# bytedance/byteps

Measured on AMD Instinct MI355X. Metric: images/sec (whole node), higher is better.
Workload: dtype bf16; 1 GPU; model=resnet50, global_batch=64, seq_len=224, parallelism=dp1, graph=True, compression=none, cross_barrier=False

## Files before the change

byteps_amd/ops/csrc/bn.hip:

```cpp
#include <hip/hip_runtime.h>
#include <hip/hip_bf16.h>

#define BLOCK 256
#define MAX_GRID 2048

namespace {

using bf16 = __hip_bfloat16;
typedef short short8 __attribute__((ext_vector_type(8)));
typedef float float4v __attribute__((ext_vector_type(4)));

__device__ inline float bf2f(bf16 v) { return __bfloat162float(v); }
__device__ inline bf16 f2bf(float v) { return __float2bfloat16(v); }

struct F8 {
  float v[8];
  __device__ void zero() {
#pragma unroll
    for (int i = 0; i < 8; ++i) v[i] = 0.0f;
  }
};

__device__ inline void load8(const bf16* p, float* out) {
  short8 r = *reinterpret_cast<const short8*>(p);
  const bf16* e = reinterpret_cast<const bf16*>(&r);
#pragma unroll
  for (int i = 0; i < 8; ++i) out[i] = bf2f(e[i]);
}

__device__ inline void store8(bf16* p, const float* in) {
  short8 r;
  bf16* e = reinterpret_cast<bf16*>(&r);
#pragma unroll
  for (int i = 0; i < 8; ++i) e[i] = f2bf(in[i]);
  *reinterpret_cast<short8*>(p) = r;
}

#define RED_BLOCKS 1024


__global__ void bn_reduce_kernel(const bf16* __restrict__ x, long long M,
                                 int C, float* __restrict__ partial) {
  const int cpt = C >> 3;
  const int groups = max(1, BLOCK / cpt);
  const int t = threadIdx.x;
  const int g = t / cpt;
  const int c8 = t - g * cpt;
  __shared__ float lds[BLOCK * 8];

  F8 s, q;
  s.zero();
  q.zero();
  if (g < groups) {
    float vals[8];
    for (long long row = (long long)blockIdx.x * groups + g; row < M;
         row += (long long)gridDim.x * groups) {
      load8(x + row * C + (c8 << 3), vals);
#pragma unroll
      for (int i = 0; i < 8; ++i) {
        s.v[i] += vals[i];
        q.v[i] += vals[i] * vals[i];
      }
    }
  }
#pragma unroll
  for (int i = 0; i < 8; ++i) lds[t * 8 + i] = s.v[i];
  __syncthreads();
  if (g == 0 && c8 < cpt) {
    for (int gg = 1; gg < groups; ++gg)
#pragma unroll
      for (int i = 0; i < 8; ++i) s.v[i] += lds[(gg * cpt + c8) * 8 + i];
#pragma unroll
    for (int i = 0; i < 8; ++i)
      partial[(long long)((c8 << 3) + i) * RED_BLOCKS + blockIdx.x] = s.v[i];
  }
  __syncthreads();
#pragma unroll
  for (int i = 0; i < 8; ++i) lds[t * 8 + i] = q.v[i];
  __syncthreads();
  if (g == 0 && c8 < cpt) {
    for (int gg = 1; gg < groups; ++gg)
#pragma unroll
      for (int i = 0; i < 8; ++i) q.v[i] += lds[(gg * cpt + c8) * 8 + i];
#pragma unroll
    for (int i = 0; i < 8; ++i)
      partial[(long long)(C + (c8 << 3) + i) * RED_BLOCKS + blockIdx.x] =
          q.v[i];
  }
}

__device__ inline float wave_row_sum(const float* __restrict__ row,
                                     int nblocks) {
  const int lane = threadIdx.x & 63;
  float acc = 0.0f;
  for (int b = lane; b < nblocks; b += 64) acc += row[b];
#pragma unroll
  for (int off = 32; off > 0; off >>= 1) acc += __shfl_down(acc, off, 64);
  return acc;
}

inline int red_grid(long long M, int C) {
  int groups = BLOCK / (C >> 3);
  if (groups < 1) groups = 1;
  long long need = (M + groups - 1) / groups;
  long long work_cap = (M * (long long)C) / 49152;
  if (work_cap < 64) work_cap = 64;
  if (need > work_cap) need = work_cap;
  if (need < 1) need = 1;
  return (int)(need < RED_BLOCKS ? need : RED_BLOCKS);
}


__global__ void bn_finalize_kernel(const float* __restrict__ partial,
                                   long long M, int C, float eps,
                                   float momentum,
                                   float* __restrict__ mean_out,
                                   float* __restrict__ invstd_out,
                                   float* __restrict__ running_mean,
                                   float* __restrict__ running_var,
                                   int update_running, int nblocks) {
  int c = blockIdx.x;
  if (c >= C) return;
  float sum = wave_row_sum(partial + (long long)c * RED_BLOCKS, nblocks);
  float sumsq = wave_row_sum(partial + (long long)(C + c) * RED_BLOCKS,
                             nblocks);
  if (threadIdx.x != 0) return;
  float n = (float)M;
  float mean = sum / n;
  float var = sumsq / n - mean * mean;
  if (var < 0.0f) var = 0.0f;
  mean_out[c] = mean;
  invstd_out[c] = rsqrtf(var + eps);
  if (update_running) {
    float unbiased = (M > 1) ? var * n / (n - 1.0f) : var;
    running_mean[c] += momentum * (mean - running_mean[c]);
    running_var[c] += momentum * (unbiased - running_var[c]);
  }
}


template <bool RELU, bool RES>
__global__ void bn_fwd_apply_kernel(const bf16* __restrict__ x,
                                    const bf16* __restrict__ res,
                                    bf16* __restrict__ y, long long M, int C,
                                    const float* __restrict__ mean,
                                    const float* __restrict__ invstd,
                                    const float* __restrict__ gamma,
                                    const float* __restrict__ beta,
                                    unsigned char* __restrict__ mask) {
  const int cpt = C >> 3;
  const long long total = M * cpt;
  for (long long idx = (long long)blockIdx.x * BLOCK + threadIdx.x;
       idx < total; idx += (long long)gridDim.x * BLOCK) {
    const long long row = idx / cpt;
    const int c8 = (int)(idx - row * cpt);
    const int c0 = c8 << 3;
    const long long off = row * C + c0;
    float vals[8], rv[8];
    load8(x + off, vals);
    if (RES) load8(res + off, rv);
    unsigned char mbits = 0;
#pragma unroll
    for (int i = 0; i < 8; ++i) {
      float scale = gamma[c0 + i] * invstd[c0 + i];
      float v = (vals[i] - mean[c0 + i]) * scale + beta[c0 + i];
      if (RES) v += rv[i];
      if (RELU) {
        if (v > 0.0f) mbits |= (unsigned char)(1u << i);
        else v = 0.0f;
      }
      vals[i] = v;
    }
    store8(y + off, vals);
    if (RELU) mask[idx] = mbits;
  }
}


template <bool RELU>
__global__ void bn_bwd_reduce_kernel(const bf16* __restrict__ x,
                                     const bf16* __restrict__ dy,
                                     const unsigned char* __restrict__ mask,
                                     long long M,
                                     int C, const float* __restrict__ mean,
                                     const float* __restrict__ invstd,
                                     float* __restrict__ partial) {
  const int cpt = C >> 3;
  const int groups = max(1, BLOCK / cpt);
  const int t = threadIdx.x;
  const int g = t / cpt;
  const int c8 = t - g * cpt;
  __shared__ float lds[BLOCK * 8];

  F8 s1, s2;
  s1.zero();
  s2.zero();
  if (g < groups) {
    float xv[8], dv[8];
    for (long long row = (long long)blockIdx.x * groups + g; row < M;
         row += (long long)gridDim.x * groups) {
      const long long off = row * C + (c8 << 3);
      load8(x + off, xv);
      load8(dy + off, dv);
      const unsigned char mbits = RELU ? mask[row * cpt + c8] : 0;
#pragma unroll
      for (int i = 0; i < 8; ++i) {
        const int c = (c8 << 3) + i;
        float dz = RELU ? ((mbits >> i) & 1 ? dv[i] : 0.0f) : dv[i];
        float xhat = (xv[i] - mean[c]) * invstd[c];
        s1.v[i] += dz;
        s2.v[i] += dz * xhat;
      }
    }
  }
#pragma unroll
  for (int i = 0; i < 8; ++i) lds[t * 8 + i] = s1.v[i];
  __syncthreads();
  if (g == 0 && c8 < cpt) {
    for (int gg = 1; gg < groups; ++gg)
#pragma unroll
      for (int i = 0; i < 8; ++i) s1.v[i] += lds[(gg * cpt + c8) * 8 + i];
#pragma unroll
    for (int i = 0; i < 8; ++i)
      partial[(long long)((c8 << 3) + i) * RED_BLOCKS + blockIdx.x] =
          s1.v[i];
  }
  __syncthreads();
#pragma unroll
  for (int i = 0; i < 8; ++i) lds[t * 8 + i] = s2.v[i];
  __syncthreads();
  if (g == 0 && c8 < cpt) {
    for (int gg = 1; gg < groups; ++gg)
#pragma unroll
      for (int i = 0; i < 8; ++i) s2.v[i] += lds[(gg * cpt + c8) * 8 + i];
#pragma unroll
    for (int i = 0; i < 8; ++i)
      partial[(long long)(C + (c8 << 3) + i) * RED_BLOCKS + blockIdx.x] =
          s2.v[i];
  }
}

__global__ void bn_fold_kernel(const float* __restrict__ partial, int C,
                               float* __restrict__ sums2, int nblocks) {
  int row = blockIdx.x;
  if (row >= 2 * C) return;
  float acc = wave_row_sum(partial + (long long)row * RED_BLOCKS, nblocks);
  if (threadIdx.x == 0) sums2[row] = acc;
}


template <bool RELU, bool RES>
__global__ void bn_bwd_apply_kernel(const bf16* __restrict__ x,
                                    const bf16* __restrict__ dy,
                                    const unsigned char* __restrict__ mask,
                                    bf16* __restrict__ dx,
                                    bf16* __restrict__ dres, long long M,
                                    int C, const float* __restrict__ mean,
                                    const float* __restrict__ invstd,
                                    const float* __restrict__ gamma,
                                    const float* __restrict__ sums2) {
  const int cpt = C >> 3;
  const long long total = M * cpt;
  const float rn = 1.0f / (float)M;
  for (long long idx = (long long)blockIdx.x * BLOCK + threadIdx.x;
       idx < total; idx += (long long)gridDim.x * BLOCK) {
    const long long row = idx / cpt;
    const int c8 = (int)(idx - row * cpt);
    const int c0 = c8 << 3;
    const long long off = row * C + c0;
    float xv[8], dv[8], dzv[8];
    load8(x + off, xv);
    load8(dy + off, dv);
    const unsigned char mbits = RELU ? mask[idx] : 0;
#pragma unroll
    for (int i = 0; i < 8; ++i) {
      const int c = c0 + i;
      float dz = RELU ? ((mbits >> i) & 1 ? dv[i] : 0.0f) : dv[i];
      dzv[i] = dz;
      float xhat = (xv[i] - mean[c]) * invstd[c];
      dv[i] = gamma[c] * invstd[c] *
              (dz - sums2[c] * rn - xhat * sums2[C + c] * rn);
    }
    store8(dx + off, dv);
    if (RES) store8(dres + off, dzv);
  }
}

inline int grid_for_rows(long long M, int C) {
  int groups = max(1, BLOCK / (C >> 3));
  long long blocks = (M + groups - 1) / groups;
  return (int)(blocks < MAX_GRID ? (blocks > 0 ? blocks : 1) : MAX_GRID);
}

inline int grid_for_elems(long long elems) {
  long long blocks = (elems + BLOCK - 1) / BLOCK;
  return (int)(blocks < MAX_GRID ? (blocks > 0 ? blocks : 1) : MAX_GRID);
}

}

#define STREAM reinterpret_cast<hipStream_t>(stream)

extern "C" {

int bps_bn_red_blocks(void) { return RED_BLOCKS; }

int bps_bn_reduce(const void* x, long long M, int C, void* partial,
                  void* stream) {
  if ((C & 7) || C > 2048) return -1;
  hipLaunchKernelGGL(bn_reduce_kernel, dim3(red_grid(M, C)), dim3(BLOCK), 0,
                     STREAM, (const bf16*)x, M, C, (float*)partial);
  return (int)hipGetLastError();
}

int bps_bn_finalize(const void* sums, long long M, int C, float eps,
                    float momentum, void* mean_out, void* invstd_out,
                    void* running_mean, void* running_var, int update_running,
                    void* stream) {
  hipLaunchKernelGGL(bn_finalize_kernel, dim3(C), dim3(64), 0,
                     STREAM, (const float*)sums, M, C, eps, momentum,
                     (float*)mean_out, (float*)invstd_out,
                     (float*)running_mean, (float*)running_var,
                     update_running, red_grid(M, C));
  return (int)hipGetLastError();
}

int bps_bn_fwd_apply(const void* x, const void* res, void* y, long long M,
                     int C, const void* mean, const void* invstd,
                     const void* gamma, const void* beta, int relu,
                     void* mask, void* stream) {
  if ((C & 7) || C > 2048) return -1;
  if (relu && !mask) return -2;
  int g = grid_for_elems(M * (C >> 3));
#define LAUNCH_FWD(R, S)                                                    \
  hipLaunchKernelGGL((bn_fwd_apply_kernel<R, S>), dim3(g), dim3(BLOCK), 0,  \
                     STREAM, (const bf16*)x, (const bf16*)res, (bf16*)y, M, \
                     C, (const float*)mean, (const float*)invstd,           \
                     (const float*)gamma, (const float*)beta,               \
                     (unsigned char*)mask)
  if (relu && res) LAUNCH_FWD(true, true);
  else if (relu) LAUNCH_FWD(true, false);
  else if (res) LAUNCH_FWD(false, true);
  else LAUNCH_FWD(false, false);
#undef LAUNCH_FWD
  return (int)hipGetLastError();
}

int bps_bn_bwd_reduce(const void* x, const void* dy, const void* mask,
                      long long M, int C, const void* mean,
                      const void* invstd, void* partial, int relu,
                      void* stream) {
  if ((C & 7) || C > 2048) return -1;
  if (relu && !mask) return -2;
  int g = red_grid(M, C);
  if (relu)
    hipLaunchKernelGGL((bn_bwd_reduce_kernel<true>), dim3(g),
                       dim3(BLOCK), 0, STREAM, (const bf16*)x,
                       (const bf16*)dy, (const unsigned char*)mask, M, C,
                       (const float*)mean, (const float*)invstd,
                       (float*)partial);
  else
    hipLaunchKernelGGL((bn_bwd_reduce_kernel<false>), dim3(g),
                       dim3(BLOCK), 0, STREAM, (const bf16*)x,
                       (const bf16*)dy, (const unsigned char*)mask, M, C,
                       (const float*)mean, (const float*)invstd,
                       (float*)partial);
  return (int)hipGetLastError();
}

int bps_bn_fold(const void* partial, long long M, int C, void* sums2,
                void* stream) {
  hipLaunchKernelGGL(bn_fold_kernel, dim3(2 * C), dim3(64), 0, STREAM,
                     (const float*)partial, C, (float*)sums2,
                     red_grid(M, C));
  return (int)hipGetLastError();
}

int bps_bn_bwd_apply(const void* x, const void* dy, const void* mask,
                     void* dx,
                     void* dres, long long M, int C, const void* mean,
                     const void* invstd, const void* gamma, const void* sums2,
                     int relu, void* stream) {
  if ((C & 7) || C > 2048) return -1;
  if (relu && !mask) return -2;
  int g = grid_for_elems(M * (C >> 3));
#define LAUNCH_BWD(R, S)                                                     \
  hipLaunchKernelGGL((bn_bwd_apply_kernel<R, S>), dim3(g), dim3(BLOCK), 0,   \
                     STREAM, (const bf16*)x, (const bf16*)dy,                \
                     (const unsigned char*)mask, (bf16*)dx, (bf16*)dres,     \
                     M, C,                                                   \
                     (const float*)mean, (const float*)invstd,               \
                     (const float*)gamma, (const float*)sums2)
  if (relu && dres) LAUNCH_BWD(true, true);
  else if (relu) LAUNCH_BWD(true, false);
  else if (dres) LAUNCH_BWD(false, true);
  else LAUNCH_BWD(false, false);
#undef LAUNCH_BWD
  return (int)hipGetLastError();
}

}
```

byteps_amd/ops/csrc/core.cc:

```cpp

#include <pybind11/pybind11.h>
#include <pybind11/stl.h>

#include <cstdint>
#include <stdexcept>

namespace py = pybind11;

extern "C" {
int bps_scale(void* x, int64_t n, float alpha, int dtype, void* stream);
int bps_cast_scale_many(const void* desc_dev, int nseg, int64_t total_vec,
                        float alpha, int src_dtype, int dst_dtype,
                        void* stream);
int bps_cast_scale(void* dst, const void* src, int64_t n, float alpha,
                   int src_dtype, int dst_dtype, void* stream);
int bps_lt_gemm_bias(const void* X, const void* W, const void* bias,
                     void* Y, int64_t M, int64_t N, int64_t K,
                     void* stream);
int bps_lt_gemm_dgelu(const void* dY2, const void* W2, const void* aux,
                      void* dY1, int64_t M, int64_t H, int64_t I,
                      void* stream);
int bps_lt_gemm_wgrad(const void* dY, const void* X, void* dW, void* db,
                      int64_t M, int64_t N, int64_t K, void* stream);
int bps_lt_gemm_dgrad(const void* dY, const void* W, void* dX, int64_t M,
                      int64_t N, int64_t K, void* stream);
int bps_axpy(void* y, const void* x, int64_t n, float alpha, int dtype,
             void* stream);
int bps_nesterov(void* g, void* m, int64_t n, float mu, int dtype,
                 void* stream);
int bps_norm(const void* x, int64_t n, int mode, void* out, int dtype,
             void* stream);
int bps_onebit_compress(const void* x, int64_t n, void* bits, void* scale_sum,
                        void* stream);
int bps_onebit_decompress(const void* bits, const void* scale_sum, int64_t n,
                          void* out, void* stream);
int bps_onebit_error(const void* x, const void* bits, const void* scale_sum,
                     int64_t n, void* err, void* stream);
int bps_randomk_compress(const void* x, int64_t n, int64_t k, uint64_t seed,
                         void* idx, void* val, void* stream);
int bps_sparse_scatter(const void* idx, const void* val, int64_t k, void* out,
                       void* stream);
int bps_sparse_error_zero(const void* idx, int64_t k, void* err, void* stream);
int bps_sparse_gather(const void* x, const void* idx, int64_t k, void* val,
                      void* stream);
int bps_dithering_compress(const void* x, int64_t n, int s, uint64_t seed,
                           int natural, const void* norm, void* code,
                           void* stream);
int bps_dithering_decompress(const void* code, int64_t n, int s, int natural,
                             const void* norm, void* out, void* stream);
int bps_fp8_compress(const void* x, int64_t n, const void* amax, void* code,
                     void* stream);
int bps_fp8_decompress(const void* code, int64_t n, const void* amax,
                       void* out, void* stream);

int bps_bn_reduce(const void* x, long long M, int C, void* sums,
                  void* stream);
int bps_bn_finalize(const void* sums, long long M, int C, float eps,
                    float momentum, void* mean_out, void* invstd_out,
                    void* running_mean, void* running_var, int update_running,
                    void* stream);
int bps_bn_fwd_apply(const void* x, const void* res, void* y, long long M,
                     int C, const void* mean, const void* invstd,
                     const void* gamma, const void* beta, int relu,
                     void* mask, void* stream);
int bps_bn_bwd_reduce(const void* x, const void* dy, const void* mask,
                      long long M, int C, const void* mean,
                      const void* invstd, void* partial, int relu,
                      void* stream);
int bps_bn_fold(const void* partial, long long M, int C, void* sums2,
                void* stream);
int bps_bn_red_blocks(void);

int bps_ln_supported(int C);
int bps_ln_red_blocks(void);
int bps_ln_fwd(const void* x, const void* gamma, const void* beta, void* y,
               long long M, int C, float eps, void* mean, void* invstd,
               void* stream);
int bps_ln_bwd(const void* x, const void* dy, const void* gamma,
               const void* mean, const void* invstd, void* dx, long long M,
               int C, void* partial, void* stream);
int bps_ln_fold(const void* partial, long long M, int C, void* sums2,
                void* stream);
int bps_bn_bwd_apply(const void* x, const void* dy, const void* mask,
                     void* dx,
                     void* dres, long long M, int C, const void* mean,
                     const void* invstd, const void* gamma, const void* sums2,
                     int relu, void* stream);

int bps_cpu_sum(void* dst, const void* src, int64_t n, int dtype);
int bps_cpu_sum2(void* dst, const void* src1, const void* src2, int64_t n,
                 float alpha, int dtype);
int bps_cpu_copy(void* dst, const void* src, int64_t nbytes);
int bps_cpu_scale(void* x, int64_t n, float alpha, int dtype);
int bps_cpu_topk_select(const float* x, int64_t n, int64_t k, int32_t* idx,
                        float* val);
int bps_cpu_dither_encode(const int8_t* code, int64_t n, uint8_t* out,
                          int64_t out_cap, int64_t* out_len);
int bps_cpu_dither_decode(const uint8_t* in, int64_t in_len, int64_t n,
                          int8_t* code);
int bps_cpu_onebit_compress(const float* x, int64_t n, uint64_t* bits,
                            float* scale_sum);
int bps_cpu_onebit_decompress(const uint64_t* bits, float scale_sum, int64_t n,
                              float* out);
int bps_cpu_randomk_indices(int64_t n, int64_t k, uint64_t seed, int32_t* idx);
int bps_cpu_sparse_scatter(const int32_t* idx, const float* val, int64_t k,
                           float* out);
int bps_cpu_sparse_accumulate(const int32_t* idx, const float* val, int64_t k,
                              float* acc);
int bps_cpu_dithering_compress(const float* x, int64_t n, int s, uint64_t seed,
                               int natural, float norm, int8_t* code);
int bps_cpu_dithering_decompress(const int8_t* code, int64_t n, int s,
                                 int natural, float norm, float* out);
int bps_cpu_fp8_compress(const float* x, int64_t n, float amax,
                         uint8_t* code);
int bps_cpu_fp8_decompress(const uint8_t* code, int64_t n, float amax,
                           float* out);
float bps_cpu_norm(const float* x, int64_t n, int mode);
}

namespace {

inline void check(int rc, const char* what) {
  if (rc != 0)
    throw std::runtime_error(std::string(what) + " failed with code " +
                             std::to_string(rc));
}

#define P(x) reinterpret_cast<void*>(static_cast<uintptr_t>(x))
#define CP(x) reinterpret_cast<const void*>(static_cast<uintptr_t>(x))

}

void init_kv(py::module_& m);
void init_server(py::module_& m);

PYBIND11_MODULE(_core, m) {
  m.doc() = "byteps_amd native core: HIP gfx950 kernels, CPU reducer, KV";
  m.attr("HIP_KERNELS") = true;

  m.def("scale", [](uintptr_t x, int64_t n, float a, int dt, uintptr_t s) {
    check(bps_scale(P(x), n, a, dt, P(s)), "bps_scale");
  });
  m.def("axpy",
        [](uintptr_t y, uintptr_t x, int64_t n, float a, int dt, uintptr_t s) {
          check(bps_axpy(P(y), CP(x), n, a, dt, P(s)), "bps_axpy");
        });
  m.def("cast_scale_many",
        [](uintptr_t desc, int nseg, int64_t total_vec, float a, int sdt,
           int ddt, uintptr_t s) {
          check(bps_cast_scale_many(CP(desc), nseg, total_vec, a, sdt, ddt,
                                    P(s)), "bps_cast_scale_many");
        });
  m.def("cast_scale",
        [](uintptr_t dst, uintptr_t src, int64_t n, float a, int sdt,
// ... 36 lines not shown
        [](uintptr_t x, int64_t n, int mode, uintptr_t out, int dt,
           uintptr_t s) {
          check(bps_norm(CP(x), n, mode, P(out), dt, P(s)), "bps_norm");
        });
  m.def("onebit_compress",
        [](uintptr_t x, int64_t n, uintptr_t bits, uintptr_t sc, uintptr_t s) {
          check(bps_onebit_compress(CP(x), n, P(bits), P(sc), P(s)),
                "bps_onebit_compress");
        });
  m.def("onebit_decompress",
        [](uintptr_t bits, uintptr_t sc, int64_t n, uintptr_t out,
           uintptr_t s) {
          check(bps_onebit_decompress(CP(bits), CP(sc), n, P(out), P(s)),
                "bps_onebit_decompress");
        });
  m.def("onebit_error",
        [](uintptr_t x, uintptr_t bits, uintptr_t sc, int64_t n, uintptr_t err,
           uintptr_t s) {
          check(bps_onebit_error(CP(x), CP(bits), CP(sc), n, P(err), P(s)),
                "bps_onebit_error");
        });
  m.def("randomk_compress",
        [](uintptr_t x, int64_t n, int64_t k, uint64_t seed, uintptr_t idx,
           uintptr_t val, uintptr_t s) {
          check(bps_randomk_compress(CP(x), n, k, seed, P(idx), P(val), P(s)),
                "bps_randomk_compress");
        });
  m.def("sparse_scatter",
        [](uintptr_t idx, uintptr_t val, int64_t k, uintptr_t out,
           uintptr_t s) {
          check(bps_sparse_scatter(CP(idx), CP(val), k, P(out), P(s)),
                "bps_sparse_scatter");
        });
  m.def("sparse_error_zero",
        [](uintptr_t idx, int64_t k, uintptr_t err, uintptr_t s) {
          check(bps_sparse_error_zero(CP(idx), k, P(err), P(s)),
                "bps_sparse_error_zero");
        });
  m.def("sparse_gather",
        [](uintptr_t x, uintptr_t idx, int64_t k, uintptr_t val, uintptr_t s) {
          check(bps_sparse_gather(CP(x), CP(idx), k, P(val), P(s)),
                "bps_sparse_gather");
        });
  m.def("dithering_compress",
        [](uintptr_t x, int64_t n, int sv, uint64_t seed, int natural,
           uintptr_t norm, uintptr_t code, uintptr_t s) {
          check(bps_dithering_compress(CP(x), n, sv, seed, natural, CP(norm),
                                       P(code), P(s)),
                "bps_dithering_compress");
        });
  m.def("dithering_decompress",
        [](uintptr_t code, int64_t n, int sv, int natural, uintptr_t norm,
           uintptr_t out, uintptr_t s) {
          check(bps_dithering_decompress(CP(code), n, sv, natural, CP(norm),
                                         P(out), P(s)),
                "bps_dithering_decompress");
        });

  m.def("fp8_compress",
        [](uintptr_t x, int64_t n, uintptr_t amax, uintptr_t code,
           uintptr_t s) {
          check(bps_fp8_compress(CP(x), n, CP(amax), P(code), P(s)),
                "bps_fp8_compress");
        });
  m.def("fp8_decompress",
        [](uintptr_t code, int64_t n, uintptr_t amax, uintptr_t out,
           uintptr_t s) {
          check(bps_fp8_decompress(CP(code), n, CP(amax), P(out), P(s)),
                "bps_fp8_decompress");
        });
  m.def("cpu_fp8_compress",
        [](uintptr_t x, int64_t n, float amax, uintptr_t code) {
          check(bps_cpu_fp8_compress((const float*)P(x), n, amax,
                                     (uint8_t*)P(code)),
                "bps_cpu_fp8_compress");
        });
  m.def("cpu_fp8_decompress",
        [](uintptr_t code, int64_t n, float amax, uintptr_t out) {
          check(bps_cpu_fp8_decompress((const uint8_t*)P(code), n, amax,
                                       (float*)P(out)),
                "bps_cpu_fp8_decompress");
        });

  m.attr("BN_RED_BLOCKS") = bps_bn_red_blocks();
  m.def("bn_reduce", [](uintptr_t x, int64_t M, int C, uintptr_t sums,
                        uintptr_t s) {
    check(bps_bn_reduce(CP(x), M, C, P(sums), P(s)), "bps_bn_reduce");
  });
  m.def("bn_fold", [](uintptr_t partial, int64_t M, int C, uintptr_t sums2,
                      uintptr_t s) {
    check(bps_bn_fold(CP(partial), M, C, P(sums2), P(s)), "bps_bn_fold");
  });
  m.def("bn_finalize",
        [](uintptr_t sums, int64_t M, int C, float eps, float momentum,
           uintptr_t mean, uintptr_t invstd, uintptr_t rmean, uintptr_t rvar,
           int upd, uintptr_t s) {
          check(bps_bn_finalize(CP(sums), M, C, eps, momentum, P(mean),
                                P(invstd), P(rmean), P(rvar), upd, P(s)),
                "bps_bn_finalize");
        });
  m.def("bn_fwd_apply",
        [](uintptr_t x, uintptr_t res, uintptr_t y, int64_t M, int C,
           uintptr_t mean, uintptr_t invstd, uintptr_t gamma, uintptr_t beta,
           int relu, uintptr_t mask, uintptr_t s) {
          check(bps_bn_fwd_apply(CP(x), CP(res), P(y), M, C, CP(mean),
                                 CP(invstd), CP(gamma), CP(beta), relu,
                                 P(mask), P(s)),
                "bps_bn_fwd_apply");
        });
  m.def("bn_bwd_reduce",
        [](uintptr_t x, uintptr_t dy, uintptr_t y, int64_t M, int C,
           uintptr_t mean, uintptr_t invstd, uintptr_t sums2, int relu,
           uintptr_t s) {
          check(bps_bn_bwd_reduce(CP(x), CP(dy), CP(y), M, C, CP(mean),
                                  CP(invstd), P(sums2), relu, P(s)),
                "bps_bn_bwd_reduce");
        });
  m.def("bn_bwd_apply",
        [](uintptr_t x, uintptr_t dy, uintptr_t y, uintptr_t dx,
           uintptr_t dres, int64_t M, int C, uintptr_t mean, uintptr_t invstd,
           uintptr_t gamma, uintptr_t sums2, int relu, uintptr_t s) {
          check(bps_bn_bwd_apply(CP(x), CP(dy), CP(y), P(dx), P(dres), M, C,
                                 CP(mean), CP(invstd), CP(gamma), CP(sums2),
                                 relu, P(s)),
                "bps_bn_bwd_apply");
        });

  m.attr("LN_RED_BLOCKS") = bps_ln_red_blocks();
  m.def("ln_supported", [](int C) { return bps_ln_supported(C) != 0; });
  m.def("ln_fwd",
        [](uintptr_t x, uintptr_t gamma, uintptr_t beta, uintptr_t y,
           int64_t M, int C, float eps, uintptr_t mean, uintptr_t invstd,
           uintptr_t s) {
          check(bps_ln_fwd(CP(x), CP(gamma), CP(beta), P(y), M, C, eps,
                           P(mean), P(invstd), P(s)),
                "bps_ln_fwd");
        });
  m.def("ln_bwd",
        [](uintptr_t x, uintptr_t dy, uintptr_t gamma, uintptr_t mean,
           uintptr_t invstd, uintptr_t dx, int64_t M, int C,
           uintptr_t partial, uintptr_t s) {
          check(bps_ln_bwd(CP(x), CP(dy), CP(gamma), CP(mean), CP(invstd),
                           P(dx), M, C, P(partial), P(s)),
                "bps_ln_bwd");
        });
  m.def("ln_fold", [](uintptr_t partial, int64_t M, int C, uintptr_t sums2,
                      uintptr_t s) {
    check(bps_ln_fold(CP(partial), M, C, P(sums2), P(s)), "bps_ln_fold");
  });

  m.def("cpu_sum", [](uintptr_t d, uintptr_t s, int64_t n, int dt) {
    check(bps_cpu_sum(P(d), CP(s), n, dt), "bps_cpu_sum");
  }, py::call_guard<py::gil_scoped_release>());
  m.def("cpu_sum2",
        [](uintptr_t d, uintptr_t a, uintptr_t b, int64_t n, float alpha,
           int dt) {
          check(bps_cpu_sum2(P(d), CP(a), CP(b), n, alpha, dt), "bps_cpu_sum2");
        }, py::call_guard<py::gil_scoped_release>());
  m.def("cpu_copy", [](uintptr_t d, uintptr_t s, int64_t nbytes) {
    check(bps_cpu_copy(P(d), CP(s), nbytes), "bps_cpu_copy");
  }, py::call_guard<py::gil_scoped_release>());
  m.def("cpu_scale", [](uintptr_t x, int64_t n, float a, int dt) {
    check(bps_cpu_scale(P(x), n, a, dt), "bps_cpu_scale");
  }, py::call_guard<py::gil_scoped_release>());
  m.def("cpu_dither_encode",
        [](uintptr_t code, int64_t n, uintptr_t out, int64_t cap) {
          int64_t wlen = 0;
          int rc = bps_cpu_dither_encode((const int8_t*)CP(code), n,
                                         (uint8_t*)P(out), cap, &wlen);
          return rc == 0 ? wlen : (int64_t)-1;
        }, py::call_guard<py::gil_scoped_release>());
  m.def("cpu_dither_decode",
        [](uintptr_t in, int64_t in_len, int64_t n, uintptr_t code) {
          check(bps_cpu_dither_decode((const uint8_t*)CP(in), in_len, n,
                                      (int8_t*)P(code)),
                "bps_cpu_dither_decode");
        }, py::call_guard<py::gil_scoped_release>());
  m.def("cpu_topk_select",
        [](uintptr_t x, int64_t n, int64_t k, uintptr_t idx, uintptr_t val) {
          check(bps_cpu_topk_select((const float*)CP(x), n, k,
                                    (int32_t*)P(idx), (float*)P(val)),
                "bps_cpu_topk_select");
        }, py::call_guard<py::gil_scoped_release>());
  m.def("cpu_onebit_compress", [](uintptr_t x, int64_t n, uintptr_t bits) {
    float sc = 0.0f;
    check(bps_cpu_onebit_compress((const float*)P(x), n, (uint64_t*)P(bits),
                                  &sc),
          "bps_cpu_onebit_compress");
    return sc;
  });
  m.def("cpu_onebit_decompress",
        [](uintptr_t bits, float sc, int64_t n, uintptr_t out) {
          check(bps_cpu_onebit_decompress((const uint64_t*)P(bits), sc, n,
                                          (float*)P(out)),
                "bps_cpu_onebit_decompress");
        });
  m.def("cpu_randomk_indices",
        [](int64_t n, int64_t k, uint64_t seed, uintptr_t idx) {
          check(bps_cpu_randomk_indices(n, k, seed, (int32_t*)P(idx)),
// ... 38 lines not shown
```

byteps_amd/torch/fused_bn.py:

```python

from __future__ import annotations

from typing import Optional

import torch
import torch.nn as nn
import torch.nn.functional as F

from .. import ops as K


def _stream(t: torch.Tensor) -> int:
    return torch.cuda.current_stream(t.device).cuda_stream


def _nhwc_ok(x: torch.Tensor, C: int) -> bool:
    return (x.is_cuda and x.dtype == torch.bfloat16 and C % 8 == 0
            and C <= 2048 and x.dim() == 4
            and x.is_contiguous(memory_format=torch.channels_last))


class _FusedBNFunction(torch.autograd.Function):
    @staticmethod
    def forward(ctx, x, residual, weight, bias, running_mean, running_var,
                momentum, eps, relu, training):
        N, C, H, W = x.shape
        M = N * H * W
        core = K.core()
        dev = x.device
        s = _stream(x)
        y = torch.empty_like(x)
        if training:
            nb = core.BN_RED_BLOCKS
            partial = torch.empty(nb * 2 * C, dtype=torch.float32,
                                  device=dev)
            core.bn_reduce(x.data_ptr(), M, C, partial.data_ptr(), s)
            mean = torch.empty(C, dtype=torch.float32, device=dev)
            invstd = torch.empty(C, dtype=torch.float32, device=dev)
            core.bn_finalize(partial.data_ptr(), M, C, eps, momentum,
                             mean.data_ptr(), invstd.data_ptr(),
                             running_mean.data_ptr(), running_var.data_ptr(),
                             1, s)
        else:
            mean = running_mean.float()
            invstd = torch.rsqrt(running_var.float() + eps)
        wf = weight.float().contiguous()
        bf = bias.float().contiguous()
        mask = torch.empty(M * (C // 8), dtype=torch.uint8, device=dev) \
            if relu else None
        core.bn_fwd_apply(x.data_ptr(),
                          residual.data_ptr() if residual is not None else 0,
                          y.data_ptr(), M, C, mean.data_ptr(),
                          invstd.data_ptr(), wf.data_ptr(), bf.data_ptr(),
                          int(relu), mask.data_ptr() if relu else 0, s)
        ctx.save_for_backward(x, mean, invstd, wf,
                              mask if mask is not None else x.new_empty(0))
        ctx.relu = relu
        ctx.has_res = residual is not None
        ctx.dims = (M, C)
        return y

    @staticmethod
    def backward(ctx, dy):
        x, mean, invstd, wf, mask = ctx.saved_tensors
        M, C = ctx.dims
        core = K.core()
        dy = dy.contiguous(memory_format=torch.channels_last)
        s = _stream(x)
        nb = core.BN_RED_BLOCKS
        mask_ptr = mask.data_ptr() if ctx.relu else 0
        partial = torch.empty(nb * 2 * C, dtype=torch.float32,
                              device=x.device)
        core.bn_bwd_reduce(x.data_ptr(), dy.data_ptr(), mask_ptr, M, C,
                           mean.data_ptr(), invstd.data_ptr(),
                           partial.data_ptr(), int(ctx.relu), s)
        sums2 = torch.empty(2 * C, dtype=torch.float32, device=x.device)
        core.bn_fold(partial.data_ptr(), M, C, sums2.data_ptr(), s)
        dx = torch.empty_like(x)
        dres = torch.empty_like(x) if ctx.has_res else None
        core.bn_bwd_apply(x.data_ptr(), dy.data_ptr(), mask_ptr,
                          dx.data_ptr(),
                          dres.data_ptr() if dres is not None else 0, M, C,
                          mean.data_ptr(), invstd.data_ptr(), wf.data_ptr(),
                          sums2.data_ptr(), int(ctx.relu), s)
        dbeta = sums2[:C]
        dgamma = sums2[C:]
        return (dx, dres, dgamma, dbeta, None, None, None, None, None, None)


class FusedBNReLU(nn.Module):

    def __init__(self, num_features: int, eps: float = 1e-5,
                 momentum: float = 0.1, relu: bool = True):
        super().__init__()
        self.num_features = num_features
        self.eps = eps
        self.momentum = momentum
        self.relu = relu
        self.weight = nn.Parameter(torch.ones(num_features))
        self.bias = nn.Parameter(torch.zeros(num_features))
        self.register_buffer("running_mean", torch.zeros(num_features))
        self.register_buffer("running_var", torch.ones(num_features))
        self.register_buffer("num_batches_tracked",
                             torch.tensor(0, dtype=torch.long))

    def forward(self, x: torch.Tensor,
                residual: Optional[torch.Tensor] = None) -> torch.Tensor:
        if _nhwc_ok(x, self.num_features) and (
                residual is None or
                residual.is_contiguous(memory_format=torch.channels_last)):
            res = residual.to(torch.bfloat16) if residual is not None else None
            return _FusedBNFunction.apply(
                x, res, self.weight, self.bias, self.running_mean,
                self.running_var, self.momentum, self.eps, self.relu,
                self.training)
        out = F.batch_norm(x, self.running_mean, self.running_var,
                           self.weight, self.bias, self.training,
                           self.momentum, self.eps)
        if residual is not None:
            out = out + residual
        return F.relu(out, inplace=True) if self.relu else out
```

Before: 5337 images/sec.

## Fuse BN stat reduction and finalize into single-pass kernels with atomic tickets

Replaces the two-kernel BN statistics path (partial reduce, then finalize/fold) with one kernel per direction. The last-arriving block, found through atomic ticket counters, performs a hierarchical fold and writes mean/invstd or the backward sums. It also tiles channels across a 2D grid (channel slices × row blocks) and unrolls the loads so several rows are in flight per iteration. This removes a kernel launch and a partial-buffer round trip per BN layer. In exchange it relies on persistent per-module ticket buffers that must reset correctly, and on memory-scope ordering between blocks, which risks races under graph capture or concurrent use.

```diff
diff --git a/byteps_amd/ops/csrc/bn.hip b/byteps_amd/ops/csrc/bn.hip
--- a/byteps_amd/ops/csrc/bn.hip
+++ b/byteps_amd/ops/csrc/bn.hip
@@ -36,106 +36,287 @@
   *reinterpret_cast<short8*>(p) = r;
 }
 
-#define RED_BLOCKS 1024
-
-
-__global__ void bn_reduce_kernel(const bf16* __restrict__ x, long long M,
-                                 int C, float* __restrict__ partial) {
+
+#define STAT_CS 16
+#define STAT_SMAX (2048 / 8 / STAT_CS)
+#define FOLD_G 16
+#define STAT_TARGET_BLOCKS 1024
+#define STAT_MIN_BLOCKS 256
+#define FWD_U 8
+#define BWD_U 4
+#define TICKET_STRIDE 32
+#define BN_TICKET_WORDS ((STAT_SMAX * FOLD_G + STAT_SMAX) * TICKET_STRIDE)
+
+typedef __attribute__((address_space(1))) unsigned gu32;
+
+struct StatGeom {
+  int cs;
+  int S;
+  int R;
+  int G;
+  int NG;
+};
+
+inline StatGeom stat_geom(long long M, int C, int U) {
+  StatGeom g;
   const int cpt = C >> 3;
-  const int groups = max(1, BLOCK / cpt);
+  g.cs = cpt < STAT_CS ? cpt : STAT_CS;
+  g.S = (cpt + g.cs - 1) / g.cs;
+  const long long groups = BLOCK / g.cs;
+  const long long per_iter = groups * U;
+  long long R = (M + per_iter - 1) / per_iter;
+  const long long want = (STAT_TARGET_BLOCKS + g.S - 1) / g.S;
+  if (R > want) R = want;
+  const long long floor_r = (STAT_MIN_BLOCKS + g.S - 1) / g.S;
+  if (R < floor_r) R = min(floor_r, (M + groups - 1) / groups);
+  if (R > FOLD_G * FOLD_G) R = FOLD_G * FOLD_G;
+  if (R < 1) R = 1;
+  g.R = (int)R;
+  g.NG = (g.R + FOLD_G - 1) / FOLD_G;
+  g.G = (g.R + g.NG - 1) / g.NG;
+  return g;
+}
+
+inline long long stat_ws_floats(const StatGeom& g) {
+  const long long nj = 16LL * g.cs;
+  return (long long)g.S * (g.R + g.NG) * nj;
+}
+
+__device__ inline void drain_vm() {
+  asm volatile("s_waitcnt vmcnt(0)" ::: "memory");
+}
+
+__device__ inline bool arrive_last(unsigned* cnt, unsigned n, float* lds,
+                                   int flag_slot) {
+  drain_vm();
+  __syncthreads();
+  if (threadIdx.x == 0) {
+    gu32* c = (gu32*)cnt;
+    const unsigned tk = __hip_atomic_fetch_add(c, 1u, __ATOMIC_RELAXED,
+                                               __HIP_MEMORY_SCOPE_AGENT);
+    const bool last = tk == n - 1;
+    if (last) {
+      __hip_atomic_store(c, 0u, __ATOMIC_RELAXED, __HIP_MEMORY_SCOPE_AGENT);
+      __builtin_amdgcn_fence(__ATOMIC_ACQUIRE, "wavefront");
+    }
+    lds[flag_slot] = last ? 1.0f : 0.0f;
+  }
+  __syncthreads();
+  return lds[flag_slot] != 0.0f;
+}
+
+__device__ inline void st_sc1(float* p, float v) {
+  __hip_atomic_store(p, v, __ATOMIC_RELAXED, __HIP_MEMORY_SCOPE_AGENT);
+}
+__device__ inline float ld_sc1(const float* p) {
+  return __hip_atomic_load(const_cast<float*>(p), __ATOMIC_RELAXED,
+                           __HIP_MEMORY_SCOPE_AGENT);
+}
+
+__device__ inline float fold_rows(const float* src, int n, int nj) {
+  float acc = 0.0f;
+  for (int k0 = 0; k0 < n; k0 += 8) {
+    float p[8];
+#pragma unroll
+    for (int u = 0; u < 8; ++u) {
+      const int k = min(k0 + u, n - 1);
+      p[u] = ld_sc1(src + (long long)k * nj);
+    }
+#pragma unroll
+    for (int u = 0; u < 8; ++u)
+      if (k0 + u < n) acc += p[u];
+  }
+  return acc;
+}
+
+__device__ inline bool stat_combine(float* lds, int groups, int nj,
+                                    float* ws, unsigned* tickets, int R,
+                                    int G, int NG) {
   const int t = threadIdx.x;
-  const int g = t / cpt;
-  const int c8 = t - g * cpt;
-  __shared__ float lds[BLOCK * 8];
+  const int slice = blockIdx.y;
+  const int rb = blockIdx.x;
+  const int flag_slot = BLOCK * 16;
+  __syncthreads();
+  float v = 0.0f;
+  if (t < nj)
+    for (int g = 0; g < groups; ++g) v += lds[g * nj + t];
+
+  float* part1 = ws + (long long)slice * R * nj;
+  if (t < nj) st_sc1(part1 + (long long)rb * nj + t, v);
+  const int grp = rb / G;
+  const int g0 = grp * G;
+  const int gn = min(G, R - g0);
+  if (!arrive_last(tickets + (slice * FOLD_G + grp) * TICKET_STRIDE, gn,
+                   lds, flag_slot))
+    return false;
+  float acc = 0.0f;
+  if (t < nj) acc = fold_rows(part1 + (long long)g0 * nj + t, gn, nj);
+
+  if (NG > 1) {
+    float* part2 = ws + (long long)gridDim.y * R * nj +
+                   (long long)slice * NG * nj;
+    if (t < nj) st_sc1(part2 + (long long)grp * nj + t, acc);
+    if (!arrive_last(tickets + (STAT_SMAX * FOLD_G + slice) * TICKET_STRIDE,
+                     NG, lds, flag_slot))
+      return false;
+    if (t < nj) acc = fold_rows(part2 + t, NG, nj);
+  }
+  if (t < nj) lds[t] = acc;
+  __syncthreads();
+  return true;
+}
+
+struct StatLane {
+  int groups, g, s, c8;
+  bool active;
+  __device__ StatLane(int cs, int cpt) {
+    groups = BLOCK / cs;
+    g = threadIdx.x / cs;
+    s = threadIdx.x - g * cs;
+    c8 = blockIdx.y * cs + s;
+    active = g < groups && c8 < cpt;
+  }
+};
+
+__device__ inline void stat_to_lds(float* lds, const StatLane& L, int cs,
+                                   const F8& a, const F8& b) {
+  if (L.g >= L.groups) return;
+  const int nj = 16 * cs;
+  float* row = lds + L.g * nj + L.s * 8;
+#pragma unroll
+  for (int i = 0; i < 8; ++i) {
+    row[i] = a.v[i];
+    row[8 * cs + i] = b.v[i];
+  }
+}
+
+template <int U>
+__global__ __launch_bounds__(BLOCK) void bn_fwd_stats_kernel(
+    const bf16* __restrict__ x, long long M, int C, float eps,
+    float momentum, float* __restrict__ mean_out,
+    float* __restrict__ invstd_out, float* __restrict__ running_mean,
+    float* __restrict__ running_var, int update_running, float* ws,
+    unsigned* tickets, int G, int NG) {
+  __shared__ float lds[BLOCK * 16 + 1];
+  const int cpt = C >> 3;
+  const int cs = min(cpt, STAT_CS);
+  const int R = gridDim.x;
+  const StatLane L(cs, cpt);
 
   F8 s, q;
   s.zero();
   q.zero();
-  if (g < groups) {
-    float vals[8];
-    for (long long row = (long long)blockIdx.x * groups + g; row < M;
-         row += (long long)gridDim.x * groups) {
-      load8(x + row * C + (c8 << 3), vals);
-#pragma unroll
-      for (int i = 0; i < 8; ++i) {
-        s.v[i] += vals[i];
-        q.v[i] += vals[i] * vals[i];
+  if (L.active) {
+    const long long stride = (long long)R * L.groups;
+    long long row = (long long)blockIdx.x * L.groups + L.g;
+    const bf16* xp = x + (L.c8 << 3);
+    for (; row < M; row += U * stride) {
+      short8 r[U];
+#pragma unroll
+      for (int u = 0; u < U; ++u) {
+        const long long rr = min(row + u * stride, M - 1);
+        r[u] = *reinterpret_cast<const short8*>(xp + rr * C);
       }
-    }
-  }
-#pragma unroll
-  for (int i = 0; i < 8; ++i) lds[t * 8 + i] = s.v[i];
-  __syncthreads();
-  if (g == 0 && c8 < cpt) {
-    for (int gg = 1; gg < groups; ++gg)
-#pragma unroll
-      for (int i = 0; i < 8; ++i) s.v[i] += lds[(gg * cpt + c8) * 8 + i];
-#pragma unroll
-    for (int i = 0; i < 8; ++i)
-      partial[(long long)((c8 << 3) + i) * RED_BLOCKS + blockIdx.x] = s.v[i];
-  }
-  __syncthreads();
-#pragma unroll
-  for (int i = 0; i < 8; ++i) lds[t * 8 + i] = q.v[i];
-  __syncthreads();
-  if (g == 0 && c8 < cpt) {
-    for (int gg = 1; gg < groups; ++gg)
-#pragma unroll
-      for (int i = 0; i < 8; ++i) q.v[i] += lds[(gg * cpt + c8) * 8 + i];
-#pragma unroll
-    for (int i = 0; i < 8; ++i)
-      partial[(long long)(C + (c8 << 3) + i) * RED_BLOCKS + blockIdx.x] =
-          q.v[i];
-  }
-}
-
-__device__ inline float wave_row_sum(const float* __restrict__ row,
-                                     int nblocks) {
-  const int lane = threadIdx.x & 63;
-  float acc = 0.0f;
-  for (int b = lane; b < nblocks; b += 64) acc += row[b];
-#pragma unroll
-  for (int off = 32; off > 0; off >>= 1) acc += __shfl_down(acc, off, 64);
-  return acc;
-}
-
-inline int red_grid(long long M, int C) {
-  int groups = BLOCK / (C >> 3);
-  if (groups < 1) groups = 1;
-  long long need = (M + groups - 1) / groups;
-  long long work_cap = (M * (long long)C) / 49152;
-  if (work_cap < 64) work_cap = 64;
-  if (need > work_cap) need = work_cap;
-  if (need < 1) need = 1;
-  return (int)(need < RED_BLOCKS ? need : RED_BLOCKS);
-}
-
-
-__global__ void bn_finalize_kernel(const float* __restrict__ partial,
-                                   long long M, int C, float eps,
-                                   float momentum,
-                                   float* __restrict__ mean_out,
-                                   float* __restrict__ invstd_out,
-                                   float* __restrict__ running_mean,
-                                   float* __restrict__ running_var,
-                                   int update_running, int nblocks) {
-  int c = blockIdx.x;
-  if (c >= C) return;
-  float sum = wave_row_sum(partial + (long long)c * RED_BLOCKS, nblocks);
-  float sumsq = wave_row_sum(partial + (long long)(C + c) * RED_BLOCKS,
-                             nblocks);
-  if (threadIdx.x != 0) return;
-  float n = (float)M;
-  float mean = sum / n;
+      __builtin_amdgcn_sched_barrier(0);
+#pragma unroll
+      for (int u = 0; u < U; ++u) {
+        const bool in = row + u * stride < M;
+        const bf16* e = reinterpret_cast<const bf16*>(&r[u]);
+#pragma unroll
+        for (int i = 0; i < 8; ++i) {
+          const float v = in ? bf2f(e[i]) : 0.0f;
+          s.v[i] += v;
+          q.v[i] += v * v;
+        }
+      }
+    }
+  }
+  stat_to_lds(lds, L, cs, s, q);
+  if (!stat_combine(lds, L.groups, 16 * cs, ws, tickets, R, G, NG)) return;
+
+  const int csw = 8 * cs;
+  const int c = threadIdx.x;
+  const int cg = blockIdx.y * csw + c;
+  if (c >= csw || cg >= C) return;
+  const float sum = lds[c];
+  const float sumsq = lds[csw + c];
+  const float n = (float)M;
+  const float mean = sum / n;
   float var = sumsq / n - mean * mean;
   if (var < 0.0f) var = 0.0f;
-  mean_out[c] = mean;
-  invstd_out[c] = rsqrtf(var + eps);
+  mean_out[cg] = mean;
+  invstd_out[cg] = rsqrtf(var + eps);
   if (update_running) {
-    float unbiased = (M > 1) ? var * n / (n - 1.0f) : var;
-    running_mean[c] += momentum * (mean - running_mean[c]);
-    running_var[c] += momentum * (unbiased - running_var[c]);
-  }
+    const float unbiased = (M > 1) ? var * n / (n - 1.0f) : var;
+    running_mean[cg] += momentum * (mean - running_mean[cg]);
+    running_var[cg] += momentum * (unbiased - running_var[cg]);
+  }
+}
+
+template <bool RELU, int U>
+__global__ __launch_bounds__(BLOCK) void bn_bwd_stats_kernel(
+    const bf16* __restrict__ x, const bf16* __restrict__ dy,
+    const unsigned char* __restrict__ mask, long long M, int C,
+    const float* __restrict__ mean, const float* __restrict__ invstd,
+    float* __restrict__ sums2, float* ws, unsigned* tickets, int G, int NG) {
+  __shared__ float lds[BLOCK * 16 + 1];
+  const int cpt = C >> 3;
+  const int cs = min(cpt, STAT_CS);
+  const int R = gridDim.x;
+  const StatLane L(cs, cpt);
+
+  F8 s1, s2;
+  s1.zero();
+  s2.zero();
+  if (L.active) {
+    const int c0 = L.c8 << 3;
+    float mu[8], is[8];
+#pragma unroll
+    for (int i = 0; i < 8; ++i) {
+      mu[i] = mean[c0 + i];
+      is[i] = invstd[c0 + i];
+    }
+    const long long stride = (long long)R * L.groups;
+    long long row = (long long)blockIdx.x * L.groups + L.g;
+    const bf16* xp = x + c0;
+    const bf16* dp = dy + c0;
+    const unsigned char* mp = mask + L.c8;
+    for (; row < M; row += U * stride) {
+      short8 xr[U], dr[U];
+      unsigned char mb[U];
+#pragma unroll
+      for (int u = 0; u < U; ++u) {
+        const long long r = min(row + u * stride, M - 1);
+        xr[u] = *reinterpret_cast<const short8*>(xp + r * C);
+        dr[u] = *reinterpret_cast<const short8*>(dp + r * C);
+        mb[u] = RELU ? mp[r * cpt] : 0;
+      }
+      __builtin_amdgcn_sched_barrier(0);
+#pragma unroll
+      for (int u = 0; u < U; ++u) {
+        const bool in = row + u * stride < M;
+        const bf16* xe = reinterpret_cast<const bf16*>(&xr[u]);
+        const bf16* de = reinterpret_cast<const bf16*>(&dr[u]);
+#pragma unroll
+        for (int i = 0; i < 8; ++i) {
+          const float dv = bf2f(de[i]);
+          const float dz = RELU ? ((mb[u] >> i) & 1 ? dv : 0.0f) : dv;
+          const float xhat = (bf2f(xe[i]) - mu[i]) * is[i];
+          s1.v[i] += in ? dz : 0.0f;
+          s2.v[i] += in ? dz * xhat : 0.0f;
+        }
+      }
+    }
+  }
+  stat_to_lds(lds, L, cs, s1, s2);
+  if (!stat_combine(lds, L.groups, 16 * cs, ws, tickets, R, G, NG)) return;
+
+  const int csw = 8 * cs;
+  const int c = threadIdx.x;
+  const int cg = blockIdx.y * csw + c;
+  if (c >= csw || cg >= C) return;
+  sums2[cg] = lds[c];
+  sums2[C + cg] = lds[csw + c];
 }
 
 
@@ -174,78 +355,6 @@
     store8(y + off, vals);
     if (RELU) mask[idx] = mbits;
   }
-}
-
-
-template <bool RELU>
-__global__ void bn_bwd_reduce_kernel(const bf16* __restrict__ x,
-                                     const bf16* __restrict__ dy,
-                                     const unsigned char* __restrict__ mask,
-                                     long long M,
-                                     int C, const float* __restrict__ mean,
-                                     const float* __restrict__ invstd,
-                                     float* __restrict__ partial) {
-  const int cpt = C >> 3;
-  const int groups = max(1, BLOCK / cpt);
-  const int t = threadIdx.x;
-  const int g = t / cpt;
-  const int c8 = t - g * cpt;
-  __shared__ float lds[BLOCK * 8];
-
-  F8 s1, s2;
-  s1.zero();
-  s2.zero();
-  if (g < groups) {
-    float xv[8], dv[8];
-    for (long long row = (long long)blockIdx.x * groups + g; row < M;
-         row += (long long)gridDim.x * groups) {
-      const long long off = row * C + (c8 << 3);
-      load8(x + off, xv);
-      load8(dy + off, dv);
-      const unsigned char mbits = RELU ? mask[row * cpt + c8] : 0;
-#pragma unroll
-      for (int i = 0; i < 8; ++i) {
-        const int c = (c8 << 3) + i;
-        float dz = RELU ? ((mbits >> i) & 1 ? dv[i] : 0.0f) : dv[i];
-        float xhat = (xv[i] - mean[c]) * invstd[c];
-        s1.v[i] += dz;
-        s2.v[i] += dz * xhat;
-      }
-    }
-  }
-#pragma unroll
-  for (int i = 0; i < 8; ++i) lds[t * 8 + i] = s1.v[i];
-  __syncthreads();
-  if (g == 0 && c8 < cpt) {
-    for (int gg = 1; gg < groups; ++gg)
-#pragma unroll
-      for (int i = 0; i < 8; ++i) s1.v[i] += lds[(gg * cpt + c8) * 8 + i];
-#pragma unroll
-    for (int i = 0; i < 8; ++i)
-      partial[(long long)((c8 << 3) + i) * RED_BLOCKS + blockIdx.x] =
-          s1.v[i];
-  }
-  __syncthreads();
-#pragma unroll
-  for (int i = 0; i < 8; ++i) lds[t * 8 + i] = s2.v[i];
-  __syncthreads();
-  if (g == 0 && c8 < cpt) {
-    for (int gg = 1; gg < groups; ++gg)
-#pragma unroll
-      for (int i = 0; i < 8; ++i) s2.v[i] += lds[(gg * cpt + c8) * 8 + i];
-#pragma unroll
-    for (int i = 0; i < 8; ++i)
-      partial[(long long)(C + (c8 << 3) + i) * RED_BLOCKS + blockIdx.x] =
-          s2.v[i];
-  }
-}
-
-__global__ void bn_fold_kernel(const float* __restrict__ partial, int C,
-                               float* __restrict__ sums2, int nblocks) {
-  int row = blockIdx.x;
-  if (row >= 2 * C) return;
-  float acc = wave_row_sum(partial + (long long)row * RED_BLOCKS, nblocks);
-  if (threadIdx.x == 0) sums2[row] = acc;
 }
 
 
@@ -303,25 +412,26 @@
 
 extern "C" {
 
-int bps_bn_red_blocks(void) { return RED_BLOCKS; }
-
-int bps_bn_reduce(const void* x, long long M, int C, void* partial,
-                  void* stream) {
-  if ((C & 7) || C > 2048) return -1;
-  hipLaunchKernelGGL(bn_reduce_kernel, dim3(red_grid(M, C)), dim3(BLOCK), 0,
-                     STREAM, (const bf16*)x, M, C, (float*)partial);
-  return (int)hipGetLastError();
-}
-
-int bps_bn_finalize(const void* sums, long long M, int C, float eps,
-                    float momentum, void* mean_out, void* invstd_out,
-                    void* running_mean, void* running_var, int update_running,
-                    void* stream) {
-  hipLaunchKernelGGL(bn_finalize_kernel, dim3(C), dim3(64), 0,
-                     STREAM, (const float*)sums, M, C, eps, momentum,
-                     (float*)mean_out, (float*)invstd_out,
+int bps_bn_ticket_words(void) { return BN_TICKET_WORDS; }
+
+long long bps_bn_stats_ws_floats(long long M, int C, int bwd) {
+  if ((C & 7) || C < 8 || C > 2048) return -1;
+  return stat_ws_floats(stat_geom(M, C, bwd ? BWD_U : FWD_U));
+}
+
+int bps_bn_fwd_stats(const void* x, long long M, int C, float eps,
+                     float momentum, void* mean_out, void* invstd_out,
+                     void* running_mean, void* running_var,
+                     int update_running, void* ws, void* tickets,
+                     void* stream) {
+  if ((C & 7) || C < 8 || C > 2048) return -1;
+  const StatGeom g = stat_geom(M, C, FWD_U);
+  hipLaunchKernelGGL((bn_fwd_stats_kernel<FWD_U>), dim3(g.R, g.S),
+                     dim3(BLOCK), 0, STREAM, (const bf16*)x, M, C, eps,
+                     momentum, (float*)mean_out, (float*)invstd_out,
                      (float*)running_mean, (float*)running_var,
-                     update_running, red_grid(M, C));
+                     update_running, (float*)ws, (unsigned*)tickets, g.G,
+                     g.NG);
   return (int)hipGetLastError();
 }
 
@@ -346,33 +456,23 @@
   return (int)hipGetLastError();
 }
 
-int bps_bn_bwd_reduce(const void* x, const void* dy, const void* mask,
-                      long long M, int C, const void* mean,
-                      const void* invstd, void* partial, int relu,
-                      void* stream) {
-  if ((C & 7) || C > 2048) return -1;
+int bps_bn_bwd_stats(const void* x, const void* dy, const void* mask,
+                     long long M, int C, const void* mean,
+                     const void* invstd, void* sums2, int relu, void* ws,
+                     void* tickets, void* stream) {
+  if ((C & 7) || C < 8 || C > 2048) return -1;
   if (relu && !mask) return -2;
-  int g = red_grid(M, C);
-  if (relu)
-    hipLaunchKernelGGL((bn_bwd_reduce_kernel<true>), dim3(g),
-                       dim3(BLOCK), 0, STREAM, (const bf16*)x,
-                       (const bf16*)dy, (const unsigned char*)mask, M, C,
-                       (const float*)mean, (const float*)invstd,
-                       (float*)partial);
-  else
-    hipLaunchKernelGGL((bn_bwd_reduce_kernel<false>), dim3(g),
-                       dim3(BLOCK), 0, STREAM, (const bf16*)x,
-                       (const bf16*)dy, (const unsigned char*)mask, M, C,
-                       (const float*)mean, (const float*)invstd,
-                       (float*)partial);
-  return (int)hipGetLastError();
-}
-
-int bps_bn_fold(const void* partial, long long M, int C, void* sums2,
-                void* stream) {
-  hipLaunchKernelGGL(bn_fold_kernel, dim3(2 * C), dim3(64), 0, STREAM,
-                     (const float*)partial, C, (float*)sums2,
-                     red_grid(M, C));
+  const StatGeom g = stat_geom(M, C, BWD_U);
+#define LAUNCH_BWD_STATS(RL)                                                 \
+  hipLaunchKernelGGL((bn_bwd_stats_kernel<RL, BWD_U>), dim3(g.R, g.S),        \
+                     dim3(BLOCK), 0, STREAM, (const bf16*)x,                 \
+                     (const bf16*)dy, (const unsigned char*)mask, M, C,      \
+                     (const float*)mean, (const float*)invstd,               \
+                     (float*)sums2, (float*)ws, (unsigned*)tickets, g.G,     \
+                     g.NG)
+  if (relu) LAUNCH_BWD_STATS(true);
+  else LAUNCH_BWD_STATS(false);
+#undef LAUNCH_BWD_STATS
   return (int)hipGetLastError();
 }
 
diff --git a/byteps_amd/ops/csrc/core.cc b/byteps_amd/ops/csrc/core.cc
--- a/byteps_amd/ops/csrc/core.cc
+++ b/byteps_amd/ops/csrc/core.cc
@@ -53,23 +53,21 @@
 int bps_fp8_decompress(const void* code, int64_t n, const void* amax,
                        void* out, void* stream);
 
-int bps_bn_reduce(const void* x, long long M, int C, void* sums,
-                  void* stream);
-int bps_bn_finalize(const void* sums, long long M, int C, float eps,
-                    float momentum, void* mean_out, void* invstd_out,
-                    void* running_mean, void* running_var, int update_running,
-                    void* stream);
+int bps_bn_ticket_words(void);
+long long bps_bn_stats_ws_floats(long long M, int C, int bwd);
+int bps_bn_fwd_stats(const void* x, long long M, int C, float eps,
+                     float momentum, void* mean_out, void* invstd_out,
+                     void* running_mean, void* running_var,
+                     int update_running, void* ws, void* tickets,
+                     void* stream);
 int bps_bn_fwd_apply(const void* x, const void* res, void* y, long long M,
                      int C, const void* mean, const void* invstd,
                      const void* gamma, const void* beta, int relu,
                      void* mask, void* stream);
-int bps_bn_bwd_reduce(const void* x, const void* dy, const void* mask,
-                      long long M, int C, const void* mean,
-                      const void* invstd, void* partial, int relu,
-                      void* stream);
-int bps_bn_fold(const void* partial, long long M, int C, void* sums2,
-                void* stream);
-int bps_bn_red_blocks(void);
+int bps_bn_bwd_stats(const void* x, const void* dy, const void* mask,
+                     long long M, int C, const void* mean,
+                     const void* invstd, void* sums2, int relu, void* ws,
+                     void* tickets, void* stream);
 
 int bps_ln_supported(int C);
 int bps_ln_red_blocks(void);
@@ -272,22 +270,20 @@
                 "bps_cpu_fp8_decompress");
         });
 
-  m.attr("BN_RED_BLOCKS") = bps_bn_red_blocks();
-  m.def("bn_reduce", [](uintptr_t x, int64_t M, int C, uintptr_t sums,
-                        uintptr_t s) {
-    check(bps_bn_reduce(CP(x), M, C, P(sums), P(s)), "bps_bn_reduce");
+  m.attr("BN_TICKET_WORDS") = bps_bn_ticket_words();
+  m.def("bn_stats_ws", [](int64_t M, int C, int bwd) {
+    long long n = bps_bn_stats_ws_floats(M, C, bwd);
+    if (n < 0) throw std::runtime_error("bn_stats_ws: unsupported C");
+    return n;
   });
-  m.def("bn_fold", [](uintptr_t partial, int64_t M, int C, uintptr_t sums2,
-                      uintptr_t s) {
-    check(bps_bn_fold(CP(partial), M, C, P(sums2), P(s)), "bps_bn_fold");
-  });
-  m.def("bn_finalize",
-        [](uintptr_t sums, int64_t M, int C, float eps, float momentum,
+  m.def("bn_fwd_stats",
+        [](uintptr_t x, int64_t M, int C, float eps, float momentum,
            uintptr_t mean, uintptr_t invstd, uintptr_t rmean, uintptr_t rvar,
-           int upd, uintptr_t s) {
-          check(bps_bn_finalize(CP(sums), M, C, eps, momentum, P(mean),
-                                P(invstd), P(rmean), P(rvar), upd, P(s)),
-                "bps_bn_finalize");
+           int upd, uintptr_t ws, uintptr_t tickets, uintptr_t s) {
+          check(bps_bn_fwd_stats(CP(x), M, C, eps, momentum, P(mean),
+                                 P(invstd), P(rmean), P(rvar), upd, P(ws),
+                                 P(tickets), P(s)),
+                "bps_bn_fwd_stats");
         });
   m.def("bn_fwd_apply",
         [](uintptr_t x, uintptr_t res, uintptr_t y, int64_t M, int C,
@@ -298,13 +294,14 @@
                                  P(mask), P(s)),
                 "bps_bn_fwd_apply");
         });
-  m.def("bn_bwd_reduce",
-        [](uintptr_t x, uintptr_t dy, uintptr_t y, int64_t M, int C,
+  m.def("bn_bwd_stats",
+        [](uintptr_t x, uintptr_t dy, uintptr_t mask, int64_t M, int C,
            uintptr_t mean, uintptr_t invstd, uintptr_t sums2, int relu,
-           uintptr_t s) {
-          check(bps_bn_bwd_reduce(CP(x), CP(dy), CP(y), M, C, CP(mean),
-                                  CP(invstd), P(sums2), relu, P(s)),
-                "bps_bn_bwd_reduce");
+           uintptr_t ws, uintptr_t tickets, uintptr_t s) {
+          check(bps_bn_bwd_stats(CP(x), CP(dy), CP(mask), M, C, CP(mean),
+                                 CP(invstd), P(sums2), relu, P(ws),
+                                 P(tickets), P(s)),
+                "bps_bn_bwd_stats");
         });
   m.def("bn_bwd_apply",
         [](uintptr_t x, uintptr_t dy, uintptr_t y, uintptr_t dx,
diff --git a/byteps_amd/torch/fused_bn.py b/byteps_amd/torch/fused_bn.py
--- a/byteps_amd/torch/fused_bn.py
+++ b/byteps_amd/torch/fused_bn.py
@@ -23,7 +23,7 @@
 class _FusedBNFunction(torch.autograd.Function):
     @staticmethod
     def forward(ctx, x, residual, weight, bias, running_mean, running_var,
-                momentum, eps, relu, training):
+                momentum, eps, relu, training, tickets):
         N, C, H, W = x.shape
         M = N * H * W
         core = K.core()
@@ -31,16 +31,14 @@
         s = _stream(x)
         y = torch.empty_like(x)
         if training:
-            nb = core.BN_RED_BLOCKS
-            partial = torch.empty(nb * 2 * C, dtype=torch.float32,
-                                  device=dev)
-            core.bn_reduce(x.data_ptr(), M, C, partial.data_ptr(), s)
+            ws = torch.empty(core.bn_stats_ws(M, C, 0), dtype=torch.float32,
+                             device=dev)
             mean = torch.empty(C, dtype=torch.float32, device=dev)
             invstd = torch.empty(C, dtype=torch.float32, device=dev)
-            core.bn_finalize(partial.data_ptr(), M, C, eps, momentum,
-                             mean.data_ptr(), invstd.data_ptr(),
-                             running_mean.data_ptr(), running_var.data_ptr(),
-                             1, s)
+            core.bn_fwd_stats(x.data_ptr(), M, C, eps, momentum,
+                              mean.data_ptr(), invstd.data_ptr(),
+                              running_mean.data_ptr(), running_var.data_ptr(),
+                              1, ws.data_ptr(), tickets.data_ptr(), s)
         else:
             mean = running_mean.float()
             invstd = torch.rsqrt(running_var.float() + eps)
@@ -58,6 +56,7 @@
         ctx.relu = relu
         ctx.has_res = residual is not None
         ctx.dims = (M, C)
+        ctx.tickets = tickets
         return y
 
     @staticmethod
@@ -67,15 +66,15 @@
         core = K.core()
         dy = dy.contiguous(memory_format=torch.channels_last)
         s = _stream(x)
-        nb = core.BN_RED_BLOCKS
         mask_ptr = mask.data_ptr() if ctx.relu else 0
-        partial = torch.empty(nb * 2 * C, dtype=torch.float32,
-                              device=x.device)
-        core.bn_bwd_reduce(x.data_ptr(), dy.data_ptr(), mask_ptr, M, C,
-                           mean.data_ptr(), invstd.data_ptr(),
-                           partial.data_ptr(), int(ctx.relu), s)
+        ws = torch.empty(core.bn_stats_ws(M, C, 1), dtype=torch.float32,
+                         device=x.device)
         sums2 = torch.empty(2 * C, dtype=torch.float32, device=x.device)
-        core.bn_fold(partial.data_ptr(), M, C, sums2.data_ptr(), s)
+        bwd_tickets = ctx.tickets.data_ptr() + 4 * core.BN_TICKET_WORDS
+        core.bn_bwd_stats(x.data_ptr(), dy.data_ptr(), mask_ptr, M, C,
+                          mean.data_ptr(), invstd.data_ptr(),
+                          sums2.data_ptr(), int(ctx.relu), ws.data_ptr(),
+                          bwd_tickets, s)
         dx = torch.empty_like(x)
         dres = torch.empty_like(x) if ctx.has_res else None
         core.bn_bwd_apply(x.data_ptr(), dy.data_ptr(), mask_ptr,
@@ -85,7 +84,8 @@
                           sums2.data_ptr(), int(ctx.relu), s)
         dbeta = sums2[:C]
         dgamma = sums2[C:]
-        return (dx, dres, dgamma, dbeta, None, None, None, None, None, None)
+        return (dx, dres, dgamma, dbeta, None, None, None, None, None, None,
+                None)
 
 
 class FusedBNReLU(nn.Module):
@@ -103,6 +103,15 @@
         self.register_buffer("running_var", torch.ones(num_features))
         self.register_buffer("num_batches_tracked",
                              torch.tensor(0, dtype=torch.long))
+        self._stat_tickets: Optional[torch.Tensor] = None
+
+    def _tickets(self, dev: torch.device) -> torch.Tensor:
+        t = self._stat_tickets
+        if t is None or t.device != dev:
+            t = torch.zeros(2 * K.core().BN_TICKET_WORDS, dtype=torch.int32,
+                            device=dev)
+            self._stat_tickets = t
+        return t
 
     def forward(self, x: torch.Tensor,
                 residual: Optional[torch.Tensor] = None) -> torch.Tensor:
@@ -113,7 +122,7 @@
             return _FusedBNFunction.apply(
                 x, res, self.weight, self.bias, self.running_mean,
                 self.running_var, self.momentum, self.eps, self.relu,
-                self.training)
+                self.training, self._tickets(x.device))
         out = F.batch_norm(x, self.running_mean, self.running_var,
                            self.weight, self.bias, self.training,
                            self.momentum, self.eps)
```

New measurement: 5770 images/sec, median of 6. +8.1%, better.
